# dalek-cryptography/curve25519-dalek

Measured on AMD Instinct MI355X. Metric: MSM scalar-mults/sec (variable-base Pippenger MSM), higher is better.
Workload: dtype u32 limbs (radix 2^25.5), u64 accumulators

## Files before the change

curve25519-dalek_amd/csrc/msm_sort.hip:

```cpp
#include <hip/hip_runtime.h>
#include <algorithm>
#include <stdlib.h>
#include <string.h>
#include <stdexcept>
#include <string>
#include <vector>
#include <functional>
#include "../../include/c25519_hip.h"
#include "devio.h"
#include "sc_sha.h"
#include "sc28.h"
#include "kernels.h"
#include "ctx.h"
#include "msm_internal.h"
#include "msm_sort.h"
#include "ffi.h"
#include "capi_util.h"

using namespace c25519;


namespace c25519 {

struct sweep_regs { u32 s[SWEEP_TPT][8]; };
typedef unsigned int sweep_u32x4 __attribute__((ext_vector_type(4)));
template <int THREADS>
__device__ __forceinline__ void sweep_load(const uint8_t *__restrict__ scalars, u64 n, u64 lo, const msm_geom &g, sweep_regs &R, u32 *__restrict__ bad_scalar, int nt) {
#pragma unroll
    for (int r = 0; r < SWEEP_TPT; r++) {
        const u64 t = lo + (u64)r * THREADS + threadIdx.x;
        u32 w[8] = {0, 0, 0, 0, 0, 0, 0, 0};
        if (t < n && nt) {
            const sweep_u32x4 *q = reinterpret_cast<const sweep_u32x4 *>(scalars) + 2 * t;
            const sweep_u32x4 a = __builtin_nontemporal_load(q), b = __builtin_nontemporal_load(q + 1);
            w[0] = a.x; w[1] = a.y; w[2] = a.z; w[3] = a.w; w[4] = b.x; w[5] = b.y; w[6] = b.z; w[7] = b.w;
        } else if (t < n) load8(scalars, t, w);
        if (bad_scalar && (w[7] >> 31)) atomicOr(bad_scalar, 1u);
        u32 carry = 0;
#pragma unroll
        for (int i = 0; i < 8; i++) { const u64 v = (u64)w[i] + g.addk[i] + carry; R.s[r][i] = (u32)v; carry = (u32)(v >> 32); }
    }
}
__device__ __forceinline__ u32 sweep_take(sweep_regs &R, int r, int wd) {
    const u32 v = R.s[r][0] & ((1u << wd) - 1u);
#pragma unroll
    for (int i = 0; i < 7; i++) R.s[r][i] = __funnelshift_r(R.s[r][i], R.s[r][i + 1], (u32)wd);
    R.s[r][7] >>= wd;
    return v;
}
template <int THREADS>
__global__ void __launch_bounds__(THREADS) k_sweep_local(const uint8_t *__restrict__ scalars, u64 n, msm_geom g, int SL, u32 *__restrict__ lsg, u32 *__restrict__ bad_blk,
                                                               u32 *__restrict__ P1, u64 wstride, u32 *__restrict__ zero_words, int nzero, int nt) {
    C25519_PRIO_CHAIN();
    extern __shared__ u32 sm[];
    constexpr int NW = THREADS / 64, CHUNK = THREADS * SWEEP_TPT;
    u32 *cnt = sm;
    u32 *cur = sm + NW * SL;
    u32 *ls = sm + 2 * NW * SL;
    u32 *stage = ls + SL + 1;
    __shared__ u32 wtot[NW];
    __shared__ u32 sbad;
    const int j = blockIdx.x, nchunk = gridDim.x, w = threadIdx.x >> 6, lane = threadIdx.x & 63;
    if (blockIdx.x == 0) for (int i = threadIdx.x; i < nzero; i += THREADS) zero_words[i] = 0;
    if (threadIdx.x == 0) sbad = 0;
    const int total = NW * SL, ept = total >= THREADS ? total / THREADS : 1;
    const int base = (int)threadIdx.x * ept;
    for (int i = threadIdx.x; i < total; i += THREADS) cnt[i] = 0;
    __syncthreads();
    const u64 lo = (u64)j * CHUNK;
    sweep_regs R;
    sweep_load<THREADS>(scalars, n, lo, g, R, &sbad, nt);
#pragma unroll 1
    for (int k = 0; k < g.nwin; k++) {
        const int wd = g.wid[k], bps = g.bps[k];
        u32 ent[SWEEP_TPT], slc[SWEEP_TPT];
#pragma unroll
        for (int r = 0; r < SWEEP_TPT; r++) {
            const u32 v = sweep_take(R, r, wd);
            slc[r] = 0xffffffffu;
            u32 sl, e;
            if (part_entry(v, k, g, bps, (u32)lo + (u32)r * THREADS + threadIdx.x, sl, e)) {
                slc[r] = sl * NW + ((u32)w ^ ((sl >> 2) & (NW - 1)));
                ent[r] = e;
                atomicAdd(&cnt[slc[r]], 1u);
            }
        }
        __syncthreads();
        u32 v4[4], tsum = 0;
#pragma unroll
        for (int e = 0; e < 4; e++) {
            v4[e] = 0;
            if (e < ept && base + e < total) { v4[e] = cnt[base + e]; cnt[base + e] = 0; }
            tsum += v4[e];
        }
        u32 inc = tsum;
        for (int off = 1; off < 64; off <<= 1) { const u32 x = __shfl_up(inc, off, 64); if (lane >= off) inc += x; }
        if (lane == 63) wtot[w] = inc;
        __syncthreads();
        u32 run = inc - tsum;
#pragma unroll
        for (int q = 0; q < NW; q++) run += q < w ? wtot[q] : 0u;
#pragma unroll
        for (int e = 0; e < 4; e++) {
            if (e < ept && base + e < total) {
                const int idx = base + e;
                cur[idx] = run;
                if ((idx & (NW - 1)) == 0) ls[idx / NW] = run;
                if (idx == total - 1) ls[SL] = run + v4[e];
            }
            run += v4[e];
        }
        __syncthreads();
#pragma unroll
        for (int r = 0; r < SWEEP_TPT; r++)
            if (slc[r] != 0xffffffffu) stage[atomicAdd(&cur[slc[r]], 1u)] = ent[r];
        __syncthreads();
        const u32 tot = ls[SL];
        u32 *dst = P1 + (u64)k * wstride + (u64)j * CHUNK;
        for (u32 i = threadIdx.x; i < tot; i += THREADS) dst[i] = stage[i];
        for (int i = threadIdx.x; i <= SL; i += THREADS) lsg[((u64)k * (SL + 1) + i) * nchunk + j] = ls[i];
    }
    if (threadIdx.x == 0) bad_blk[j] = sbad;
}
__global__ void __launch_bounds__(256) k_bin_totals(const u32 *__restrict__ lsg, int nchunk, int SL, int nbins, u32 *__restrict__ binm, const u32 *__restrict__ bad_blk,
                                                    u32 *__restrict__ bad_ws, u32 *__restrict__ bad_sticky) {
    C25519_PRIO_CHAIN();
    if (blockIdx.x == 0) {
        u32 any = 0;
        for (int i = threadIdx.x; i < nchunk; i += 256) any |= bad_blk[i];
        any = __syncthreads_or((int)any);
        if (threadIdx.x == 0) { *bad_ws = any ? 1u : 0u; if (any && bad_sticky) atomicOr(bad_sticky, 1u); }
    }
    const int bin = blockIdx.x * 4 + (threadIdx.x >> 6), lane = threadIdx.x & 63;
    if (bin >= nbins) return;
    const int k = bin / SL, s = bin % SL;
    const u32 *row0 = lsg + ((u64)k * (SL + 1) + s) * nchunk, *row1 = row0 + nchunk;
    u32 sum = 0;
    for (int j = lane; j < nchunk; j += 64) sum += row1[j] - row0[j];
#pragma unroll
    for (int d = 32; d > 0; d >>= 1) sum += (u32)__shfl_xor((int)sum, d, 64);
    if (lane == 0) binm[bin] = sum;
}


template <int NW, int ITER>
__global__ void __launch_bounds__(64 * NW) __attribute__((amdgpu_waves_per_eu(NW / 2, NW / 2)))
k_part2g(const u32 *__restrict__ P1, u64 n, u64 wstride, u32 chunk, msm_geom g, int SL, int nchunk, const u32 *__restrict__ lsg, const u32 *__restrict__ binm,
         u32 *__restrict__ totals, u32 *__restrict__ base, u32 *__restrict__ sorted,
         u32 *__restrict__ ord_hist, u32 max_items, long_item *__restrict__ items, u32 *__restrict__ counters,
         u32 *__restrict__ long_gids, u32 *__restrict__ long_first) {
    C25519_PRIO_CHAIN();
    extern __shared__ u32 sm[];
    u32 *cnt = sm, *cur = sm + PART_BPS_MAX, *oh = sm + 2 * PART_BPS_MAX, *out = sm + 3 * PART_BPS_MAX, *wl = out + PART_CAP;
    __shared__ u32 red[NW], red_all[NW];
    const int k = blockIdx.x, sidx = blockIdx.y, tid = threadIdx.x, lane = tid & 63, w = tid >> 6;
    const int PART_BPS = 1 << g.bps[k], sh = part_entry_shift(g);
    const u32 *row0 = lsg + ((u64)k * (SL + 1) + sidx) * nchunk, *row1 = row0 + nchunk;
    const u32 *src = P1 + (u64)k * wstride;
    const u32 mine = tid < SL ? binm[(u64)k * SL + tid] : 0u;
    u32 part = tid < sidx ? mine : 0u, all = mine;
    const u32 m = binm[(u64)k * SL + sidx];
    if (tid < PART_BPS) cnt[tid] = 0;
    if (tid < 256) oh[tid] = 0;
    int nslots = 0;
    for (int j0 = 0; j0 < nchunk; j0 += NW * 64) {
        const int j = j0 + w + NW * lane;
        u32 st = 0, len = 0;
        if (j < nchunk) { st = row0[j]; len = row1[j] - st; }
        const u32 np = (len + 63u) >> 6;
        u32 inc = np;
        for (int off = 1; off < 64; off <<= 1) { const u32 x = __shfl_up(inc, off, 64); if (lane >= off) inc += x; }
        const u32 first = (u32)nslots + inc - np;
        for (u32 p = 0; p < np; p++)
            if (first + p < (u32)ITER) wl[w * ITER + first + p] = (((u32)j * chunk + st + 64u * p) << 7) | (len - 64u * p < 64u ? len - 64u * p : 64u);
        nslots += (int)__shfl(inc, 63, 64);
    }
#pragma unroll
    for (int d = 32; d > 0; d >>= 1) { part += (u32)__shfl_xor((int)part, d, 64); all += (u32)__shfl_xor((int)all, d, 64); }
    if (lane == 0) { red[w] = part; red_all[w] = all; }
    const bool fits = !__syncthreads_or(nslots > ITER) && m <= (u32)PART_CAP;
    u32 b0 = 0, wtot = 0;
#pragma unroll
    for (int q = 0; q < NW; q++) { b0 += red[q]; wtot += red_all[q]; }
    if (sidx == SL - 1 && tid == 0) base[(u64)k * (g.half + 1) + g.half] = wtot;
    {
        const int per = (1 << g.bps_log2) - PART_BPS, first = (SL << g.bps[k]) + sidx * per;
        for (int i = tid; i < per; i += 64 * NW) { totals[(u64)k * g.half + first + i] = 0; base[(u64)k * (g.half + 1) + first + i] = wtot; }
        if (per > 0 && tid == 0) atomicAdd(&ord_hist[256 * msm_group_of(g, k) + 255], (u32)per);
    }
    u32 *dst = sorted + (u64)k * n + b0;
    if (fits) {
#pragma unroll 1
        for (int t0 = 0; t0 < nslots; t0 += 8) {
            u32 ev[8];
            bool ok[8];
#pragma unroll
            for (int q = 0; q < 8; q++) {
                const u32 d = t0 + q < nslots ? wl[w * ITER + t0 + q] : 0u;
                ok[q] = (u32)lane < (d & 127u);
                ev[q] = ok[q] ? src[(d >> 7) + lane] : 0u;
            }
#pragma unroll
            for (int q = 0; q < 8; q++) if (ok[q]) atomicAdd(&cnt[ev[q] >> sh], 1u);
        }
    } else {
        for (int j = w; j < nchunk; j += NW) {
            const u32 st = row0[j], en = row1[j];
            for (u32 o = st + lane; o < en; o += 64) atomicAdd(&cnt[src[(u64)j * chunk + o] >> sh], 1u);
        }
    }
    __syncthreads();
    if (tid < 64) {
        const int per = PART_BPS >> 6;
        u32 c4[8] = {0, 0, 0, 0, 0, 0, 0, 0}, sum = 0;
        for (int q = 0; q < per; q++) { c4[q] = cnt[per * tid + q]; sum += c4[q]; }
        u32 inc = sum;
        for (int off = 1; off < 64; off <<= 1) { u32 x = __shfl_up(inc, off, 64); if (tid >= off) inc += x; }
        u32 run = inc - sum;
        for (int q = 0; q < per; q++) { cur[per * tid + q] = run; run += c4[q]; }
    }
    __syncthreads();
    if (tid < PART_BPS) {
        const u64 b = (u64)sidx * PART_BPS + tid;
        totals[(u64)k * g.half + b] = cnt[tid];
        base[(u64)k * (g.half + 1) + b] = b0 + cur[tid];
    }
    __syncthreads();
    if (tid < PART_BPS) order_note_bucket(cnt[tid], (u64)k * g.half + (u64)sidx * PART_BPS + tid, g, base, oh, max_items, items, counters, long_gids, long_first);
    __syncthreads();
    if (tid < 256 && oh[tid]) atomicAdd(&ord_hist[256 * msm_group_of(g, k) + tid], oh[tid]);
    if (fits) {
#pragma unroll 1
        for (int t0 = 0; t0 < nslots; t0 += 8) {
            u32 ev[8];
            bool ok[8];
#pragma unroll
            for (int q = 0; q < 8; q++) {
                const u32 d = t0 + q < nslots ? wl[w * ITER + t0 + q] : 0u;
                ok[q] = (u32)lane < (d & 127u);
                ev[q] = ok[q] ? src[(d >> 7) + lane] : 0u;
            }
#pragma unroll
            for (int q = 0; q < 8; q++) if (ok[q]) out[atomicAdd(&cur[ev[q] >> sh], 1u)] = part_entry_final(ev[q], sh);
        }
        __syncthreads();
        for (u32 i = tid; i < m; i += 64 * NW) dst[i] = out[i];
    } else {
        for (int j = w; j < nchunk; j += NW) {
            const u32 st = row0[j], en = row1[j];
            for (u32 o0 = st; o0 < en; o0 += 64) {
                const u32 o = o0 + lane;
                const bool have = o < en;
                const u32 ev = have ? src[(u64)j * chunk + o] : 0u, bk = ev >> sh;
                const u32 lead_bk = __shfl(bk, __ffsll((long long)__ballot(have)) - 1, 64);
                const unsigned long long same = __ballot(have && bk == lead_bk);
                u32 pos = 0;
                if (have && bk == lead_bk) {
                    const int leader = __ffsll((long long)same) - 1;
                    u32 first = 0;
                    if (lane == leader) first = atomicAdd(&cur[bk], (u32)__popcll(same));
                    first = __shfl(first, leader, 64);
                    pos = first + (u32)__popcll(same & ((1ull << lane) - 1ull));
                } else if (have) {
                    pos = atomicAdd(&cur[bk], 1u);
                }
                if (have) dst[pos] = part_entry_final(ev, sh);
            }
        }
    }
}

template <int BS>
__global__ void __launch_bounds__(BS) k_order_place(const u32 *__restrict__ totals, u64 nb, const u32 *__restrict__ ord_hist, u32 *__restrict__ ord_cursor, u32 *__restrict__ perm, msm_geom g) {
    C25519_PRIO_CHAIN();
    __shared__ u32 h[256], start[256], basep[256];
    const int lane = threadIdx.x & 63, w = threadIdx.x >> 6;
    const int grp = g.ngroups > 1 ? msm_group_of(g, (int)(((u64)blockIdx.x * BS) / (u64)g.half)) : 0;
    ord_hist += 256 * grp; ord_cursor += 256 * grp; perm += (u64)g.gstart[grp] * (u64)g.half;
    if (threadIdx.x < 256) {
        const u32 mine = ord_hist[threadIdx.x];
        u32 inc = mine;
        for (int off = 1; off < 64; off <<= 1) { const u32 y = __shfl_up(inc, off, 64); if (lane >= off) inc += y; }
        h[threadIdx.x] = 0;
        if (lane == 63) basep[w] = inc;
        start[threadIdx.x] = inc - mine;
    }
    __syncthreads();
    if (threadIdx.x < 256) {
        u32 wb = 0;
        for (int i = 0; i < w; i++) wb += basep[i];
        start[threadIdx.x] += wb;
    }
    const u64 gid = (u64)blockIdx.x * BS + threadIdx.x;
    u32 bin = 0, local = 0;
    if (gid < nb) { const u32 c = totals[gid]; bin = 255u - (c > 255u ? 255u : c); local = atomicAdd(&h[bin], 1u); }
    __syncthreads();
    if (threadIdx.x < 256 && h[threadIdx.x]) basep[threadIdx.x] = start[threadIdx.x] + atomicAdd(&ord_cursor[threadIdx.x], h[threadIdx.x]);
    __syncthreads();
    if (gid < nb) perm[basep[bin] + local] = (u32)gid;
}

}

using namespace c25519;

void launch_order_place(const uint32_t *totals, uint64_t nb, const uint32_t *ord_hist, uint32_t *ord_cursor, uint32_t *perm, const c25519::msm_geom &g, hipStream_t st) {
    hipLaunchKernelGGL(k_order_place<1024>, dim3(div_up64(nb, 1024)), dim3(1024), 0, st, totals, nb, ord_hist, ord_cursor, perm, g);
}

void msm_slice_params(msm_geom &g) {
    int lsl = 0; while ((g.half >> g.bps_log2) > (1 << lsl)) lsl++;
    for (int k = 0; k < MSM_MAX_WIN; k++) {
        const int bits = k < g.nwin ? (k < g.first_unsigned ? g.wid[k] - 1 : g.wid[k]) : 0;
        int b = bits - lsl;
        if (b < 6) b = 6;
        if (b > g.bps_log2) b = g.bps_log2;
        g.bps[k] = (unsigned char)b;
    }
}
void msm_sort_params(uint64_t n, msm_geom &g) {
    g.bps_log2 = (g.half > (1 << 15) && n <= (1ull << 22)) ? 9 : 8;
    while (g.bps_log2 > 6 && (n << g.bps_log2) / (uint64_t)g.half > 16500) g.bps_log2--;
    if ((1 << g.bps_log2) > g.half) { g.bps_log2 = 0; while ((2 << g.bps_log2) <= g.half) g.bps_log2++; }
    const uint64_t mean = n / (uint64_t)g.half + 1;
    g.long_cap = (u32)std::max<uint64_t>(LONG_CAP_MIN, (mean * 5 + 1) / 2);
}

int32_t msm_enqueue_sort(c25519_ctx *ctx, const uint8_t *d_scalars, uint64_t n_scalars, const msm_geom &g, uint32_t *d_slot, hipStream_t sort_stream, msm_plan &pl,
                         const msm_merged *md, uint64_t n_carve, hipEvent_t lists_free, int parity) {
    (void)d_slot;
    const uint64_t n = md ? (uint64_t)md->K * md->ns : n_scalars;
    const uint64_t nc = n_carve > n ? n_carve : n;
    if (!md && (g.half < 64 || n > (1ull << (part_entry_shift(g) - 1)))) return bad_arg(ctx, "msm: internal error (a pass outside the range of the chunk-local sort)");
    static const uint64_t chunk_local_min = (uint64_t)C25519_KNOB("SORT_CHUNK_LOCAL_MIN", 1 << 16);
    const bool matrix = md != nullptr || nc < chunk_local_min;
    int nchunk = std::max(1, std::min(64, 512 / g.nwin));
    while (nchunk > 1 && nc / nchunk < 4096) nchunk /= 2;
    if ((nc + nchunk - 1) / nchunk > 65536) nchunk = (int)((nc + 65535) / 65536);
    const uint64_t nb = (uint64_t)g.nwin * g.half;
    const int nseg = red_nseg(g.half);
    size_t off = 0;
    auto carve = [&](size_t bytes) { size_t o = off; off += (bytes + 255) & ~(size_t)255; return o; };
    const int copies = parity >= 0 ? 2 : 1, cp = parity >= 0 ? (parity & 1) : 0;
    const size_t szB = ((size_t)g.nwin * (g.half + 1) * 4 + 255) & ~(size_t)255, szS = ((size_t)g.nwin * nc * 4 + 255) & ~(size_t)255, szPerm = (nb * 4 + 255) & ~(size_t)255;
    const size_t oD = carve(matrix ? (size_t)g.nwin * nc * 2 : 0), oC = carve(matrix ? (size_t)g.nwin * nchunk * g.half * 4 : 0), oB = carve(szB * copies) + szB * cp;
    const size_t oS = carve(szS * copies) + szS * cp, oK = carve(nb * 160), oT = carve(nb * 4);
    const size_t oSW = carve((size_t)g.nwin * nseg * 2 * 160), oF = carve(16384), oPerm = carve(szPerm * copies) + szPerm * cp;
    const uint64_t entries = (uint64_t)g.nwin * nc;
    const uint32_t max_long = (uint32_t)std::min<uint64_t>(nb, entries / g.long_cap + 1);
    const uint32_t max_items = (uint32_t)(entries / LONG_SEG + max_long + 1);
    const size_t oLI = carve((size_t)max_items * sizeof(long_item)), oLG = carve((size_t)max_long * 4), oLF = carve((size_t)max_long * 4);
    const size_t oLS = carve((size_t)max_items * 160);
    const bool use_part = matrix && g.c >= 13 && n <= (1ull << 23) && n >= (1ull << 16);
    static const int small_blocks = C25519_KNOB("SORT_SMALL", 0);
    static const int sweep_threads = small_blocks ? 256 : (C25519_KNOB("SWEEP_THREADS", SWEEP_THREADS) == 512 ? 512 : SWEEP_THREADS);
    const int sweep_chunk = sweep_threads * SWEEP_TPT;
    const int SL = std::max(1, g.half >> g.bps_log2), PART_CHUNK = matrix ? part_chunk(SL) : sweep_chunk, pchunks = (int)((n + PART_CHUNK - 1) / PART_CHUNK), pchunks_c = (int)((nc + PART_CHUNK - 1) / PART_CHUNK);
    const size_t p1_words = matrix ? (size_t)g.nwin * nc : (size_t)g.nwin * pchunks_c * sweep_chunk;
    size_t oP1 = 0, oCC = 0, oBB = 0;
    if (!matrix || use_part) { oP1 = carve(p1_words * 4); oCC = carve((size_t)g.nwin * (SL + 1) * pchunks_c * 4); oBB = carve((size_t)g.nwin * (SL + 1) * 4 + (size_t)pchunks_c * 4); }
    int32_t r = ctx_reserve(ctx, ctx->tmp_d, off);
    if (r) return r;
    uint8_t *ws = (uint8_t *)ctx->tmp_d.p;
    uint32_t *base = (uint32_t *)(ws + oB), *sorted = (uint32_t *)(ws + oS), *buckets = (uint32_t *)(ws + oK);
    uint32_t *flags = (uint32_t *)(ws + oF), *totals = (uint32_t *)(ws + oT), *ord_hist = flags + 64, *perm = (uint32_t *)(ws + oPerm);
    const int ngr = g.ngroups > 1 ? g.ngroups : 1;
    uint32_t *ord_cursor = flags + 64 + 256 * ngr, *bad_ws = flags + 64 + 512 * ngr;
    const int ZERO_WORDS = 64 + 512 * ngr;
    if (ngr > 1 && (matrix || g.half < 1024)) return bad_arg(ctx, "msm: internal error (window groups outside the chunk-local sort)");
    pl.g = g; pl.n = n; pl.nb = nb; pl.nseg = nseg; pl.max_items = max_items; pl.max_long = max_long;
    pl.base = base; pl.sorted = sorted; pl.buckets = buckets; pl.perm = perm; pl.SW = (uint32_t *)(ws + oSW); pl.counters = flags + 8; pl.bad_ws = bad_ws;
    pl.items = (long_item *)(ws + oLI); pl.lgids = (uint32_t *)(ws + oLG); pl.lfirst = (uint32_t *)(ws + oLF); pl.segs = (uint32_t *)(ws + oLS);
    pl.sort_stream = sort_stream;
    hipStream_t st = sort_stream ? sort_stream : ctx->stream;
    if (matrix) {
        if (lists_free) HIPCHK(hipStreamWaitEvent(st, lists_free, 0));
        msm_matrix_sort_args a;
        a.d_scalars = d_scalars; a.n_scalars = n_scalars; a.n = n; a.nchunk = nchunk; a.use_part = use_part; a.SL = SL; a.PART_CHUNK = PART_CHUNK; a.pchunks = pchunks;
        a.D = (uint16_t *)(ws + oD); a.counts = (uint32_t *)(ws + oC); a.P1 = (uint32_t *)(ws + oP1); a.cc = (uint32_t *)(ws + oCC); a.bin_base = (uint32_t *)(ws + oBB);
        a.flags = flags; a.totals = totals; a.ord_hist = ord_hist;
        return msm_matrix_sort_enqueue(ctx, g, md, pl, a, st);
    }
    uint32_t *P1 = (uint32_t *)(ws + oP1), *lsg = (uint32_t *)(ws + oCC), *binm = (uint32_t *)(ws + oBB), *bad_blk = binm + (size_t)g.nwin * (SL + 1);
    const uint64_t wstride = (uint64_t)pchunks_c * sweep_chunk;
    constexpr int ITER_SMALL = 160;
    const int nw1 = sweep_chunk / SWEEP_TPT / 64;
    const size_t lds1 = ((size_t)2 * nw1 * SL + SL + 1 + sweep_chunk) * 4;
    const size_t lds2 = ((size_t)3 * PART_BPS_MAX + PART_CAP + (small_blocks ? 8 * ITER_SMALL : 16 * P2G_ITER)) * 4;
    static const int sweep_nt = C25519_KNOB("SWEEP_NT", 0);
    if (small_blocks) {
        HIPCHK(hipFuncSetAttribute(reinterpret_cast<const void *>(k_sweep_local<256>), hipFuncAttributeMaxDynamicSharedMemorySize, (int)lds1));
        HIPCHK(hipFuncSetAttribute(reinterpret_cast<const void *>(k_part2g<8, ITER_SMALL>), hipFuncAttributeMaxDynamicSharedMemorySize, (int)lds2));
        hipLaunchKernelGGL(k_sweep_local<256>, dim3(pchunks), dim3(256), lds1, st, d_scalars, n, g, SL, lsg, bad_blk, P1, wstride, flags, ZERO_WORDS, sweep_nt);
    } else if (sweep_threads == 512) {
        HIPCHK(hipFuncSetAttribute(reinterpret_cast<const void *>(k_part2g<16, P2G_ITER>), hipFuncAttributeMaxDynamicSharedMemorySize, (int)lds2));
        hipLaunchKernelGGL(k_sweep_local<512>, dim3(pchunks), dim3(512), lds1, st, d_scalars, n, g, SL, lsg, bad_blk, P1, wstride, flags, ZERO_WORDS, sweep_nt);
    } else {
        HIPCHK(hipFuncSetAttribute(reinterpret_cast<const void *>(k_sweep_local<SWEEP_THREADS>), hipFuncAttributeMaxDynamicSharedMemorySize, (int)lds1));
        HIPCHK(hipFuncSetAttribute(reinterpret_cast<const void *>(k_part2g<16, P2G_ITER>), hipFuncAttributeMaxDynamicSharedMemorySize, (int)lds2));
        hipLaunchKernelGGL(k_sweep_local<SWEEP_THREADS>, dim3(pchunks), dim3(SWEEP_THREADS), lds1, st, d_scalars, n, g, SL, lsg, bad_blk, P1, wstride, flags, ZERO_WORDS, sweep_nt);
    }
    hipLaunchKernelGGL(k_bin_totals, dim3((g.nwin * SL + 3) / 4), dim3(256), 0, st, lsg, pchunks, SL, g.nwin * SL, binm, bad_blk, bad_ws, pl.bad_sticky);
    if (pl.ev_partition) HIPCHK(hipEventRecord(pl.ev_partition, st));
    if (lists_free) HIPCHK(hipStreamWaitEvent(st, lists_free, 0));
    if (small_blocks) hipLaunchKernelGGL((k_part2g<8, ITER_SMALL>), dim3(g.nwin, SL), dim3(512), lds2, st, P1, n, wstride, (u32)sweep_chunk, g, SL, pchunks, lsg, binm, totals, base, sorted, ord_hist, max_items, pl.items, pl.counters, pl.lgids, pl.lfirst);
    else hipLaunchKernelGGL((k_part2g<16, P2G_ITER>), dim3(g.nwin, SL), dim3(1024), lds2, st, P1, n, wstride, (u32)sweep_chunk, g, SL, pchunks, lsg, binm, totals, base, sorted, ord_hist, max_items, pl.items, pl.counters, pl.lgids, pl.lfirst);
    hipLaunchKernelGGL(k_order_place<1024>, dim3(div_up64(nb, 1024)), dim3(1024), 0, st, totals, nb, ord_hist, ord_cursor, perm, g);
    HIPCHK(hipGetLastError());
    return C25519_OK;
}
```

Baseline: 1.296 billion.

## Fuse bin totals into part2g, drop second LDS atomic pass, batch order_place

The sweep kernel now reserves each entry's slot with the first counting atomic and packs the slot, local rank and entry bits into one register. This removes the second atomicAdd pass over a separate cursor array and double-buffers the count arrays so the reset happens once. The k_bin_totals kernel is removed: k_part2g computes the per-bin prefix and size from the lsg rows itself and also performs the bad-block reduction, which saves one launch and one global pass. k_order_place gains an items-per-thread template so it can launch four times fewer blocks, with a fallback when the group geometry is not aligned. The bit packing assumes small per-bin counts (fewer than 1024) and limited entry width, which could be fragile.

Result: no change. 1.294 billion (median of 6 runs) (-0.2%).

```diff
diff --git a/curve25519-dalek_amd/csrc/msm_sort.hip b/curve25519-dalek_amd/csrc/msm_sort.hip
--- a/curve25519-dalek_amd/csrc/msm_sort.hip
+++ b/curve25519-dalek_amd/csrc/msm_sort.hip
@@ -54,18 +54,17 @@
     C25519_PRIO_CHAIN();
     extern __shared__ u32 sm[];
     constexpr int NW = THREADS / 64, CHUNK = THREADS * SWEEP_TPT;
-    u32 *cnt = sm;
-    u32 *cur = sm + NW * SL;
+    u32 *cnt0 = sm;
     u32 *ls = sm + 2 * NW * SL;
     u32 *stage = ls + SL + 1;
     __shared__ u32 wtot[NW];
     __shared__ u32 sbad;
-    const int j = blockIdx.x, nchunk = gridDim.x, w = threadIdx.x >> 6, lane = threadIdx.x & 63;
+    const int j = blockIdx.x, nchunk = gridDim.x, w = threadIdx.x >> 6, lane = threadIdx.x & 63, sh = part_entry_shift(g);
     if (blockIdx.x == 0) for (int i = threadIdx.x; i < nzero; i += THREADS) zero_words[i] = 0;
     if (threadIdx.x == 0) sbad = 0;
     const int total = NW * SL, ept = total >= THREADS ? total / THREADS : 1;
     const int base = (int)threadIdx.x * ept;
-    for (int i = threadIdx.x; i < total; i += THREADS) cnt[i] = 0;
+    for (int i = threadIdx.x; i < 2 * total; i += THREADS) cnt0[i] = 0;
     __syncthreads();
     const u64 lo = (u64)j * CHUNK;
     sweep_regs R;
@@ -73,16 +72,16 @@
 #pragma unroll 1
     for (int k = 0; k < g.nwin; k++) {
         const int wd = g.wid[k], bps = g.bps[k];
-        u32 ent[SWEEP_TPT], slc[SWEEP_TPT];
+        u32 *cnt = cnt0 + (k & 1) * total, *nxt = cnt0 + ((k & 1) ^ 1) * total;
+        u32 slc[SWEEP_TPT];
 #pragma unroll
         for (int r = 0; r < SWEEP_TPT; r++) {
             const u32 v = sweep_take(R, r, wd);
             slc[r] = 0xffffffffu;
             u32 sl, e;
-            if (part_entry(v, k, g, bps, (u32)lo + (u32)r * THREADS + threadIdx.x, sl, e)) {
-                slc[r] = sl * NW + ((u32)w ^ ((sl >> 2) & (NW - 1)));
-                ent[r] = e;
-                atomicAdd(&cnt[slc[r]], 1u);
+            if (part_entry(v, k, g, bps, 0u, sl, e)) {
+                const u32 c = sl * NW + ((u32)w ^ ((sl >> 2) & (NW - 1)));
+                slc[r] = c << 20 | atomicAdd(&cnt[c], 1u) << 10 | e >> (sh - 1);
             }
         }
         __syncthreads();
@@ -90,7 +89,7 @@
 #pragma unroll
         for (int e = 0; e < 4; e++) {
             v4[e] = 0;
-            if (e < ept && base + e < total) { v4[e] = cnt[base + e]; cnt[base + e] = 0; }
+            if (e < ept && base + e < total) { v4[e] = cnt[base + e]; nxt[base + e] = 0; }
             tsum += v4[e];
         }
         u32 inc = tsum;
@@ -104,7 +103,7 @@
         for (int e = 0; e < 4; e++) {
             if (e < ept && base + e < total) {
                 const int idx = base + e;
-                cur[idx] = run;
+                cnt[idx] = run;
                 if ((idx & (NW - 1)) == 0) ls[idx / NW] = run;
                 if (idx == total - 1) ls[SL] = run + v4[e];
             }
@@ -113,7 +112,8 @@
         __syncthreads();
 #pragma unroll
         for (int r = 0; r < SWEEP_TPT; r++)
-            if (slc[r] != 0xffffffffu) stage[atomicAdd(&cur[slc[r]], 1u)] = ent[r];
+            if (slc[r] != 0xffffffffu)
+                stage[cnt[slc[r] >> 20] + ((slc[r] >> 10) & 1023u)] = (slc[r] & 1023u) << (sh - 1) | ((u32)lo + (u32)r * THREADS + threadIdx.x);
         __syncthreads();
         const u32 tot = ls[SL];
         u32 *dst = P1 + (u64)k * wstride + (u64)j * CHUNK;
@@ -122,51 +122,38 @@
     }
     if (threadIdx.x == 0) bad_blk[j] = sbad;
 }
-__global__ void __launch_bounds__(256) k_bin_totals(const u32 *__restrict__ lsg, int nchunk, int SL, int nbins, u32 *__restrict__ binm, const u32 *__restrict__ bad_blk,
-                                                    u32 *__restrict__ bad_ws, u32 *__restrict__ bad_sticky) {
-    C25519_PRIO_CHAIN();
-    if (blockIdx.x == 0) {
-        u32 any = 0;
-        for (int i = threadIdx.x; i < nchunk; i += 256) any |= bad_blk[i];
-        any = __syncthreads_or((int)any);
-        if (threadIdx.x == 0) { *bad_ws = any ? 1u : 0u; if (any && bad_sticky) atomicOr(bad_sticky, 1u); }
-    }
-    const int bin = blockIdx.x * 4 + (threadIdx.x >> 6), lane = threadIdx.x & 63;
-    if (bin >= nbins) return;
-    const int k = bin / SL, s = bin % SL;
-    const u32 *row0 = lsg + ((u64)k * (SL + 1) + s) * nchunk, *row1 = row0 + nchunk;
-    u32 sum = 0;
-    for (int j = lane; j < nchunk; j += 64) sum += row1[j] - row0[j];
-#pragma unroll
-    for (int d = 32; d > 0; d >>= 1) sum += (u32)__shfl_xor((int)sum, d, 64);
-    if (lane == 0) binm[bin] = sum;
-}
-
-
 template <int NW, int ITER>
 __global__ void __launch_bounds__(64 * NW) __attribute__((amdgpu_waves_per_eu(NW / 2, NW / 2)))
-k_part2g(const u32 *__restrict__ P1, u64 n, u64 wstride, u32 chunk, msm_geom g, int SL, int nchunk, const u32 *__restrict__ lsg, const u32 *__restrict__ binm,
+k_part2g(const u32 *__restrict__ P1, u64 n, u64 wstride, u32 chunk, msm_geom g, int SL, int nchunk, const u32 *__restrict__ lsg,
+         const u32 *__restrict__ bad_blk, u32 *__restrict__ bad_ws, u32 *__restrict__ bad_sticky,
          u32 *__restrict__ totals, u32 *__restrict__ base, u32 *__restrict__ sorted,
          u32 *__restrict__ ord_hist, u32 max_items, long_item *__restrict__ items, u32 *__restrict__ counters,
          u32 *__restrict__ long_gids, u32 *__restrict__ long_first) {
     C25519_PRIO_CHAIN();
     extern __shared__ u32 sm[];
     u32 *cnt = sm, *cur = sm + PART_BPS_MAX, *oh = sm + 2 * PART_BPS_MAX, *out = sm + 3 * PART_BPS_MAX, *wl = out + PART_CAP;
-    __shared__ u32 red[NW], red_all[NW];
+    __shared__ u32 red[NW], red_all[NW], red_m[NW];
     const int k = blockIdx.x, sidx = blockIdx.y, tid = threadIdx.x, lane = tid & 63, w = tid >> 6;
     const int PART_BPS = 1 << g.bps[k], sh = part_entry_shift(g);
-    const u32 *row0 = lsg + ((u64)k * (SL + 1) + sidx) * nchunk, *row1 = row0 + nchunk;
+    if (k == 0 && sidx == 0) {
+        u32 any = 0;
+        for (int i = tid; i < nchunk; i += 64 * NW) any |= bad_blk[i];
+        any = __syncthreads_or((int)any);
+        if (tid == 0) { *bad_ws = any ? 1u : 0u; if (any && bad_sticky) atomicOr(bad_sticky, 1u); }
+    }
+    const u32 *row0 = lsg + ((u64)k * (SL + 1) + sidx) * nchunk, *row1 = row0 + nchunk, *rowT = lsg + ((u64)k * (SL + 1) + SL) * nchunk;
     const u32 *src = P1 + (u64)k * wstride;
-    const u32 mine = tid < SL ? binm[(u64)k * SL + tid] : 0u;
-    u32 part = tid < sidx ? mine : 0u, all = mine;
-    const u32 m = binm[(u64)k * SL + sidx];
+    const int per = (1 << g.bps_log2) - PART_BPS;
+    const bool want_all = per > 0 && sidx != SL - 1;
+    u32 part = 0, all = 0, mm = 0;
     if (tid < PART_BPS) cnt[tid] = 0;
     if (tid < 256) oh[tid] = 0;
     int nslots = 0;
     for (int j0 = 0; j0 < nchunk; j0 += NW * 64) {
         const int j = j0 + w + NW * lane;
         u32 st = 0, len = 0;
-        if (j < nchunk) { st = row0[j]; len = row1[j] - st; }
+        if (j < nchunk) { st = row0[j]; len = row1[j] - st; if (want_all) all += rowT[j]; }
+        part += st; mm += len;
         const u32 np = (len + 63u) >> 6;
         u32 inc = np;
         for (int off = 1; off < 64; off <<= 1) { const u32 x = __shfl_up(inc, off, 64); if (lane >= off) inc += x; }
@@ -176,15 +163,19 @@
         nslots += (int)__shfl(inc, 63, 64);
     }
 #pragma unroll
-    for (int d = 32; d > 0; d >>= 1) { part += (u32)__shfl_xor((int)part, d, 64); all += (u32)__shfl_xor((int)all, d, 64); }
-    if (lane == 0) { red[w] = part; red_all[w] = all; }
-    const bool fits = !__syncthreads_or(nslots > ITER) && m <= (u32)PART_CAP;
-    u32 b0 = 0, wtot = 0;
-#pragma unroll
-    for (int q = 0; q < NW; q++) { b0 += red[q]; wtot += red_all[q]; }
+    for (int d = 32; d > 0; d >>= 1) {
+        part += (u32)__shfl_xor((int)part, d, 64); all += (u32)__shfl_xor((int)all, d, 64); mm += (u32)__shfl_xor((int)mm, d, 64);
+    }
+    if (lane == 0) { red[w] = part; red_all[w] = all; red_m[w] = mm; }
+    const bool over = __syncthreads_or(nslots > ITER);
+    u32 b0 = 0, wtot = 0, m = 0;
+#pragma unroll
+    for (int q = 0; q < NW; q++) { b0 += red[q]; wtot += red_all[q]; m += red_m[q]; }
+    if (!want_all) wtot = b0 + m;
+    const bool fits = !over && m <= (u32)PART_CAP;
     if (sidx == SL - 1 && tid == 0) base[(u64)k * (g.half + 1) + g.half] = wtot;
     {
-        const int per = (1 << g.bps_log2) - PART_BPS, first = (SL << g.bps[k]) + sidx * per;
+        const int first = (SL << g.bps[k]) + sidx * per;
         for (int i = tid; i < per; i += 64 * NW) { totals[(u64)k * g.half + first + i] = 0; base[(u64)k * (g.half + 1) + first + i] = wtot; }
         if (per > 0 && tid == 0) atomicAdd(&ord_hist[256 * msm_group_of(g, k) + 255], (u32)per);
     }
@@ -270,12 +261,13 @@
     }
 }
 
-template <int BS>
+template <int BS, int IPT>
 __global__ void __launch_bounds__(BS) k_order_place(const u32 *__restrict__ totals, u64 nb, const u32 *__restrict__ ord_hist, u32 *__restrict__ ord_cursor, u32 *__restrict__ perm, msm_geom g) {
     C25519_PRIO_CHAIN();
     __shared__ u32 h[256], start[256], basep[256];
     const int lane = threadIdx.x & 63, w = threadIdx.x >> 6;
-    const int grp = g.ngroups > 1 ? msm_group_of(g, (int)(((u64)blockIdx.x * BS) / (u64)g.half)) : 0;
+    const u64 blo = (u64)blockIdx.x * BS * IPT;
+    const int grp = g.ngroups > 1 ? msm_group_of(g, (int)(blo / (u64)g.half)) : 0;
     ord_hist += 256 * grp; ord_cursor += 256 * grp; perm += (u64)g.gstart[grp] * (u64)g.half;
     if (threadIdx.x < 256) {
         const u32 mine = ord_hist[threadIdx.x];
@@ -291,13 +283,21 @@
         for (int i = 0; i < w; i++) wb += basep[i];
         start[threadIdx.x] += wb;
     }
-    const u64 gid = (u64)blockIdx.x * BS + threadIdx.x;
-    u32 bin = 0, local = 0;
-    if (gid < nb) { const u32 c = totals[gid]; bin = 255u - (c > 255u ? 255u : c); local = atomicAdd(&h[bin], 1u); }
+    u32 bin[IPT], local[IPT];
+#pragma unroll
+    for (int i = 0; i < IPT; i++) {
+        const u64 gid = blo + (u64)i * BS + threadIdx.x;
+        bin[i] = 0; local[i] = 0;
+        if (gid < nb) { const u32 c = totals[gid]; bin[i] = 255u - (c > 255u ? 255u : c); local[i] = atomicAdd(&h[bin[i]], 1u); }
+    }
     __syncthreads();
     if (threadIdx.x < 256 && h[threadIdx.x]) basep[threadIdx.x] = start[threadIdx.x] + atomicAdd(&ord_cursor[threadIdx.x], h[threadIdx.x]);
     __syncthreads();
-    if (gid < nb) perm[basep[bin] + local] = (u32)gid;
+#pragma unroll
+    for (int i = 0; i < IPT; i++) {
+        const u64 gid = blo + (u64)i * BS + threadIdx.x;
+        if (gid < nb) perm[basep[bin[i]] + local[i]] = (u32)gid;
+    }
 }
 
 }
@@ -305,7 +305,7 @@
 using namespace c25519;
 
 void launch_order_place(const uint32_t *totals, uint64_t nb, const uint32_t *ord_hist, uint32_t *ord_cursor, uint32_t *perm, const c25519::msm_geom &g, hipStream_t st) {
-    hipLaunchKernelGGL(k_order_place<1024>, dim3(div_up64(nb, 1024)), dim3(1024), 0, st, totals, nb, ord_hist, ord_cursor, perm, g);
+    hipLaunchKernelGGL((k_order_place<1024, 1>), dim3(div_up64(nb, 1024)), dim3(1024), 0, st, totals, nb, ord_hist, ord_cursor, perm, g);
 }
 
 void msm_slice_params(msm_geom &g) {
@@ -381,7 +381,7 @@
         a.flags = flags; a.totals = totals; a.ord_hist = ord_hist;
         return msm_matrix_sort_enqueue(ctx, g, md, pl, a, st);
     }
-    uint32_t *P1 = (uint32_t *)(ws + oP1), *lsg = (uint32_t *)(ws + oCC), *binm = (uint32_t *)(ws + oBB), *bad_blk = binm + (size_t)g.nwin * (SL + 1);
+    uint32_t *P1 = (uint32_t *)(ws + oP1), *lsg = (uint32_t *)(ws + oCC), *bad_blk = (uint32_t *)(ws + oBB);
     const uint64_t wstride = (uint64_t)pchunks_c * sweep_chunk;
     constexpr int ITER_SMALL = 160;
     const int nw1 = sweep_chunk / SWEEP_TPT / 64;
@@ -400,12 +400,12 @@
         HIPCHK(hipFuncSetAttribute(reinterpret_cast<const void *>(k_part2g<16, P2G_ITER>), hipFuncAttributeMaxDynamicSharedMemorySize, (int)lds2));
         hipLaunchKernelGGL(k_sweep_local<SWEEP_THREADS>, dim3(pchunks), dim3(SWEEP_THREADS), lds1, st, d_scalars, n, g, SL, lsg, bad_blk, P1, wstride, flags, ZERO_WORDS, sweep_nt);
     }
-    hipLaunchKernelGGL(k_bin_totals, dim3((g.nwin * SL + 3) / 4), dim3(256), 0, st, lsg, pchunks, SL, g.nwin * SL, binm, bad_blk, bad_ws, pl.bad_sticky);
     if (pl.ev_partition) HIPCHK(hipEventRecord(pl.ev_partition, st));
     if (lists_free) HIPCHK(hipStreamWaitEvent(st, lists_free, 0));
-    if (small_blocks) hipLaunchKernelGGL((k_part2g<8, ITER_SMALL>), dim3(g.nwin, SL), dim3(512), lds2, st, P1, n, wstride, (u32)sweep_chunk, g, SL, pchunks, lsg, binm, totals, base, sorted, ord_hist, max_items, pl.items, pl.counters, pl.lgids, pl.lfirst);
-    else hipLaunchKernelGGL((k_part2g<16, P2G_ITER>), dim3(g.nwin, SL), dim3(1024), lds2, st, P1, n, wstride, (u32)sweep_chunk, g, SL, pchunks, lsg, binm, totals, base, sorted, ord_hist, max_items, pl.items, pl.counters, pl.lgids, pl.lfirst);
-    hipLaunchKernelGGL(k_order_place<1024>, dim3(div_up64(nb, 1024)), dim3(1024), 0, st, totals, nb, ord_hist, ord_cursor, perm, g);
+    if (small_blocks) hipLaunchKernelGGL((k_part2g<8, ITER_SMALL>), dim3(g.nwin, SL), dim3(512), lds2, st, P1, n, wstride, (u32)sweep_chunk, g, SL, pchunks, lsg, bad_blk, bad_ws, pl.bad_sticky, totals, base, sorted, ord_hist, max_items, pl.items, pl.counters, pl.lgids, pl.lfirst);
+    else hipLaunchKernelGGL((k_part2g<16, P2G_ITER>), dim3(g.nwin, SL), dim3(1024), lds2, st, P1, n, wstride, (u32)sweep_chunk, g, SL, pchunks, lsg, bad_blk, bad_ws, pl.bad_sticky, totals, base, sorted, ord_hist, max_items, pl.items, pl.counters, pl.lgids, pl.lfirst);
+    if (g.ngroups <= 1 || g.half % 4096 == 0) hipLaunchKernelGGL((k_order_place<1024, 4>), dim3(div_up64(nb, 4096)), dim3(1024), 0, st, totals, nb, ord_hist, ord_cursor, perm, g);
+    else hipLaunchKernelGGL((k_order_place<1024, 1>), dim3(div_up64(nb, 1024)), dim3(1024), 0, st, totals, nb, ord_hist, ord_cursor, perm, g);
     HIPCHK(hipGetLastError());
     return C25519_OK;
 }
```
